# q8888620002/Group-Attribution-for-Diffusion-Models

Measured on AMD Instinct MI355X. Metric: shapley_coalitions_per_hour, higher is better.
Workload: dtype f32; 1 GPU; CIFAR-20 DDPM sFT coalition (BASELINE configs[1]): gd_steps=1000 @B=128 + 10240 samples x 100 DDIM steps @B=32 (32 batches fused/launch), UNet2DModel widths [128, 256, 256, 256] 35.75M params fp32; step = 1/1000 coalition = 1 train step + 1 sampler step @B=1024, enqueued on 3 HIP streams (the train step belongs to a later coalition: independent work); coalitions_in_flight=3

## Files before the change

group-attribution-for-diffusion-models_amd/csrc/gemm_f32.hip:

```cpp
#include "gad_common.h"
#include "gemm_dev.h"

using namespace gadk;

namespace gadk {
void launch_wino4_fused(const DevArgs& w, int bm, hipStream_t st);
}

namespace {

template <int ROWS, int VEC>
struct LoadKCDense : KCSlots<ROWS> {
  using S = KCSlots<ROWS>;
  const float* base;
  long roff[S::NS];
  unsigned rowmask;
  int kend, k;
  bool kok;
  __device__ void init(const float* b, int ld, int row0, int nrows, int kend_) {
    base = b;
    kend = kend_;
    rowmask = 0;
#pragma unroll
    for (int i = 0; i < S::NS; ++i) {
      int r = row0 + S::row(i);
      bool ok = r < nrows;
      roff[i] = ok ? (long)r * ld : 0;
      rowmask |= (unsigned)ok << i;
    }
  }
  __device__ __forceinline__ void prep(int k0, unsigned& mask) {
    k = k0 + S::kq4();
    kok = k < kend;
    mask = rowmask;
// ... 2470 lines not shown
static bool use_wino_wgrad(const gad_gemm_args* a, WinoWgradPlan* wq) {
  const gad_conv_geom& g = a->g;
  if (!(a->flags & GAD_GEMM_WINO_WGRAD) || (a->flags & (GAD_GEMM_NO_WINO | GAD_GEMM_NO_PATCH | GAD_GEMM_INTERNAL_WINO4))) return false;
  if (a->operand_precision != 0 || a->a_mode != GAD_A_MC || a->b_mode != GAD_B_CONV || a->A2 || a->A_k2 || a->batch > 1) return false;
  if (!same_3x3(g) || (g.Ho & 3) || (g.Wo & 3)) return false;
  if (g.C % 4 != 0 || g.ldx % 4 != 0 || a->M % 4 != 0 || a->lda % 4 != 0 || a->N != 9 * g.C || a->ldc % 4 != 0) return false;
  if ((a->tile_hint != 0 && a->tile_hint != HINT_WINO4) || a->splitk_hint > 0 || a->K % (g.Ho * g.Wo) != 0) return false;
  if (a->alpha != 1.f || a->bias || a->rowadd || a->residual) return false;
  if (!(gad_aligned16(a->A) && gad_aligned16(a->B) && gad_aligned16(a->C))) return false;
  wq->T = (long)a->K / 16;
  wq->wy_bytes = (int64_t)36 * wq->T * a->M * 4;
  wq->v_bytes = (int64_t)36 * wq->T * g.C * 4;
  wq->du_bytes = (int64_t)36 * a->M * g.C * 4;
  wq->bytes = wq->wy_bytes + wq->v_bytes + wq->du_bytes;
  if (a->tile_hint == HINT_WINO4) return true;
  const double dy_bytes = 4.0 * a->K * a->M, x_bytes = 4.0 * (double)(a->K / (g.Ho * g.Wo)) * g.H * g.W * g.C;
  const double t_w = (dy_bytes + x_bytes + (double)wq->wy_bytes + (double)wq->v_bytes) / 4.9e12 + 36.0 * wq->T * a->M * (double)g.C * 2.0 / 100e12 +
                     3.0 * (double)wq->du_bytes / 3.0e12 + 30e-6;
  const double t_direct = 2.0 * a->K * (double)a->M * a->N / 115e12;
  return t_w < 0.9 * t_direct;
}


static gad_gemm_args products36(const gad_gemm_args* a, const float* A, const float* B, float* C, int am, int bm, int M, int N, int K) {
  gad_gemm_args sub = *a;
  sub.A = A; sub.B = B; sub.C = C;
  sub.a_mode = am; sub.b_mode = bm;
  sub.M = M; sub.N = N; sub.K = K;
  sub.lda = am == GAD_A_MC ? M : K; sub.ldb = bm == GAD_B_MC ? N : K; sub.ldc = N;
  sub.batch = 36; sub.batch_inner = 1;
  sub.strideA0 = (int64_t)M * K; sub.strideB0 = (int64_t)N * K; sub.strideC0 = (int64_t)M * N;
  sub.strideA1 = sub.strideB1 = sub.strideC1 = 0;
  sub.tile_hint = 0; sub.splitk_hint = 0;
  sub.flags = GAD_GEMM_INTERNAL_WINO4;
  sub.B_wino = nullptr; sub.B_wino4 = nullptr; sub.wino_ws = nullptr; sub.wino_ws_bytes = 0;
  sub.A2 = nullptr;
  return sub;
}
static gad_gemm_args wino_wgrad_products_args(const gad_gemm_args* a, const WinoWgradPlan& wq, float* Wy, float* V, float* dU) {
  return products36(a, Wy, V, dU, GAD_A_MC, GAD_B_MC, a->M, a->g.C, (int)wq.T);
}
static gad_gemm_args wino4_products_args(const gad_gemm_args* a, const WinoPlan& wp, float* V, float* Mb) {
  gad_gemm_args sub = products36(a, V, a->B_wino4, Mb, GAD_A_KC, GAD_B_KC, (int)wp.T, a->N, a->g.C);
  sub.alpha = 1.f; sub.bias = nullptr; sub.rowadd = nullptr; sub.residual = nullptr;
  return sub;
}

enum class RouteKind { ENGINE, PATCH_F32, PATCH_BF16, FEWOUT, WGRAD_PATCH, WINO, WINO_WGRAD, SPLIT_N, SPLIT_M };
struct Route {
  RouteKind kind;
  gad_gemm_args a;
  int vec;
  bool bf16;
  Plan plan;
  PatchPlan pp;
  WinoPlan wp;
  WinoWgradPlan wq;
  int wbm, wsplits;
  int split;
};

static Route route_of(const gad_gemm_args* args) {
  Route r{};
  r.a = canonical(args);
  const gad_gemm_args* a = &r.a;
  r.vec = pick_vec(a);
  r.bf16 = use_bf16(a);
  if (use_wino_wgrad(a, &r.wq)) r.kind = RouteKind::WINO_WGRAD;
  else if (use_wino(a, &r.wp)) r.kind = RouteKind::WINO;
  else if (patch_split_n(a, &r.split)) {
    r.kind = RouteKind::SPLIT_N;
    use_patch_conv_f32(a, &r.pp);
  } else if (wgrad_split_m(a, &r.split)) {
    r.kind = RouteKind::SPLIT_M;
    r.wsplits = wgrad_patch_splits(a, &r.wbm);
  } else if (use_fewout_conv(a)) r.kind = RouteKind::FEWOUT;
  else if ((r.wsplits = wgrad_patch_splits(a, &r.wbm))) r.kind = RouteKind::WGRAD_PATCH;
  else if (use_patch_conv(a)) r.kind = RouteKind::PATCH_BF16;
  else if (use_patch_conv_f32(a, &r.pp)) r.kind = RouteKind::PATCH_F32;
  else {
    r.kind = RouteKind::ENGINE;
    r.plan = make_plan(a);
  }
  return r;
}

struct Report { int kid, tile, splitk; };
static Report report(const Route& r) {
  switch (r.kind) {
    case RouteKind::ENGINE: return {r.bf16 ? 1 : 0, r.plan.bm, r.plan.splitk};
    case RouteKind::PATCH_F32: return {2, r.pp.bn, r.pp.splitk};
    case RouteKind::SPLIT_N: return {2, 224, r.pp.splitk};
    case RouteKind::SPLIT_M: return {2, 224, r.wsplits};
    case RouteKind::WGRAD_PATCH: return {2, r.wbm, r.wsplits};
    case RouteKind::PATCH_BF16: return {3, 128, 1};
    case RouteKind::FEWOUT: return {4, 256, 1};
    case RouteKind::WINO: return {r.wp.f == 2 ? 5 : 6, r.wp.f == 2 ? r.wp.bn : (r.wp.fused4 == 2 ? r.wp.bm : 128), 1};
    case RouteKind::WINO_WGRAD: return {7, 128, 1};
  }
  return {-1, 0, 0};
}

static void split_halves(const Route& r, gad_gemm_args* lo, gad_gemm_args* hi) {
  const gad_gemm_args* a = &r.a;
  const int s = r.split;
  *lo = *a;
  *hi = *a;
  if (r.kind == RouteKind::SPLIT_M) {
    if (a->tile_hint >= HINT_SPLIT_M) lo->tile_hint = hi->tile_hint = 0;
    lo->M = s;
    hi->M = a->M - s;
    hi->A = a->A + s;
    hi->C = a->C + (long)s * a->ldc;
    return;
  }
  lo->B_wino = lo->B_wino4 = hi->B_wino = hi->B_wino4 = nullptr;
  lo->wino_ws = hi->wino_ws = nullptr;
  lo->wino_ws_bytes = hi->wino_ws_bytes = 0;
  lo->N = s;
  hi->N = a->N - s;
  hi->B = a->B + (long)s * a->ldb;
  hi->C = a->C + s;
  if (a->bias) hi->bias = a->bias + s;
  if (a->rowadd) hi->rowadd = a->rowadd + s;
  if (a->residual) hi->residual = a->residual + s;
}

static int64_t workspace_bytes(const Route& r) {
  const gad_gemm_args* a = &r.a;
  switch (r.kind) {
    case RouteKind::ENGINE: case RouteKind::PATCH_F32: case RouteKind::WGRAD_PATCH: case RouteKind::PATCH_BF16: case RouteKind::FEWOUT: {
      const int splitk = report(r).splitk;
      return splitk > 1 ? (int64_t)(a->batch > 0 ? a->batch : 1) * splitk * a->M * a->N * (int64_t)sizeof(float) : 0;
    }
    case RouteKind::WINO: {
      if (r.wp.f == 2 || r.wp.fused4) return 0;
      const gad_gemm_args sub = wino4_products_args(a, r.wp, nullptr, nullptr);
      return gad_gemm_workspace_bytes(&sub);
    }
    case RouteKind::WINO_WGRAD: {
      const gad_gemm_args sub = wino_wgrad_products_args(a, r.wq, nullptr, nullptr, nullptr);
      return gad_gemm_workspace_bytes(&sub);
    }
    case RouteKind::SPLIT_N: case RouteKind::SPLIT_M: {
      gad_gemm_args lo, hi;
      split_halves(r, &lo, &hi);
      const int64_t wl = gad_gemm_workspace_bytes(&lo), wh = gad_gemm_workspace_bytes(&hi);
      return wl > wh ? wl : wh;
    }
  }
  return 0;
}

extern "C" int gad_gemm_uses_bf16(const gad_gemm_args* a) { return a && route_of(a).bf16 ? 1 : 0; }

extern "C" int gad_gemm_kernel_id(const gad_gemm_args* a) { return a ? report(route_of(a)).kid : -1; }

extern "C" int gad_gemm_plan(const gad_gemm_args* a, int32_t* tile, int32_t* splitk, int32_t* vec) {
  GAD_CHECK(a && tile && splitk && vec, "gad_gemm_plan: null pointer");
  const Route r = route_of(a);
  const Report rep = report(r);
  *tile = rep.tile;
  *splitk = rep.splitk;
  *vec = r.vec;
  return 0;
}

extern "C" int64_t gad_gemm_wino_bytes(const gad_gemm_args* a) {
  if (!a) return 0;
  const Route r = route_of(a);
  return r.kind == RouteKind::WINO ? r.wp.bytes : r.kind == RouteKind::WINO_WGRAD ? r.wq.bytes : 0;
}

extern "C" int64_t gad_gemm_workspace_bytes(const gad_gemm_args* a) { return a ? workspace_bytes(route_of(a)) : 0; }

extern "C" int gad_wino_weights(const float* src, float* dst, const int64_t* table, int64_t n_tiles, void* stream) {
// ... 384 lines not shown
  GAD_CASE(GAD_A_MC, GAD_B_MC)
  GAD_CASE(GAD_A_CONV, GAD_B_KC)
  GAD_CASE(GAD_A_CONVT, GAD_B_WDGRAD)
  GAD_CASE(GAD_A_MC, GAD_B_CONV)
  {
    gad_set_error("gad_gemm: unsupported mode pair a_mode=%d b_mode=%d", am, bmode);
    return 1;
  }
#undef GAD_CASE
  GAD_LAUNCH_CHECK("gad_gemm");
  if (pl.splitk > 1) {
    launch_splitk_reduce(d, (int)batch, st);
    GAD_LAUNCH_CHECK("gad_gemm(splitk reduce)");
  }
  return 0;
}

extern "C" int gad_gemm(const gad_gemm_args* args, void* stream) {
  GAD_CHECK(args && args->A && args->B && args->C, "gad_gemm: null pointer");
  const gad_gemm_args canon = canonical(args);
  if (const int rc = check_args(&canon)) return rc;
  const Route r = route_of(&canon);
  if (const int rc = check_stage_flags(r)) return rc;
  hipStream_t st = (hipStream_t)stream;
  DevArgs d = dev_args(&r.a);
  switch (r.kind) {
    case RouteKind::SPLIT_N: case RouteKind::SPLIT_M: {
      gad_gemm_args lo, hi;
      split_halves(r, &lo, &hi);
      const int rc = gad_gemm(&lo, stream);
      return rc ? rc : gad_gemm(&hi, stream);
    }
    case RouteKind::WINO_WGRAD: return launch_wino_wgrad(r, stream);
    case RouteKind::WINO: return launch_wino(r, d, stream);
    case RouteKind::FEWOUT: return launch_fewout(r, d, st);
    case RouteKind::WGRAD_PATCH: return launch_wgrad_patch(r, d, st);
    case RouteKind::PATCH_BF16: return launch_patch_bf16(r, d, st);
    case RouteKind::PATCH_F32: return launch_patch_f32(r, d, st);
    case RouteKind::ENGINE: return launch_engine(r, d, st);
  }
  return 1;
}
```

group-attribution-for-diffusion-models_amd/gad/_capi.py:

```python
import ctypes as C
import os

_HERE = os.path.dirname(os.path.abspath(__file__))
LIB_PATH = os.path.join(_HERE, "libgad_hip.so")


class GadError(RuntimeError):
    pass


class ConvGeom(C.Structure):
    _fields_ = [("H", C.c_int32), ("W", C.c_int32), ("C", C.c_int32), ("ldx", C.c_int32),
                ("Ho", C.c_int32), ("Wo", C.c_int32), ("KH", C.c_int32), ("KW", C.c_int32),
                ("stride", C.c_int32), ("pad_t", C.c_int32), ("pad_l", C.c_int32), ("upsample", C.c_int32)]


class GemmArgs(C.Structure):
    _fields_ = [("A", C.c_void_p), ("B", C.c_void_p), ("C", C.c_void_p),
                ("a_mode", C.c_int32), ("b_mode", C.c_int32),
                ("M", C.c_int32), ("N", C.c_int32), ("K", C.c_int32),
                ("lda", C.c_int32), ("ldb", C.c_int32), ("ldc", C.c_int32),
                ("batch", C.c_int32), ("batch_inner", C.c_int32),
                ("strideA0", C.c_int64), ("strideA1", C.c_int64), ("strideB0", C.c_int64),
                ("strideB1", C.c_int64), ("strideC0", C.c_int64), ("strideC1", C.c_int64),
# ... 48 lines not shown
                ("ws", C.c_void_p), ("ws_bytes", C.c_int64),
                ("tile_hint", C.c_int32), ("splitk_hint", C.c_int32)]


class AdamArgs(C.Structure):
    _fields_ = [("p", C.c_void_p), ("g", C.c_void_p), ("m", C.c_void_p), ("v", C.c_void_p), ("ema", C.c_void_p),
                ("n", C.c_int64), ("sumsq", C.c_void_p), ("max_norm", C.c_float),
                ("lr", C.c_float), ("beta1", C.c_float), ("beta2", C.c_float), ("eps", C.c_float),
                ("weight_decay", C.c_float), ("adamw", C.c_int32), ("step", C.c_int32), ("ema_decay", C.c_float)]


class JLArgs(C.Structure):
    _fields_ = [("A", C.c_void_p), ("lda", C.c_int64), ("G", C.c_int32), ("P", C.c_int64), ("p0", C.c_int64),
                ("d", C.c_int32), ("seed", C.c_uint32), ("model_id", C.c_uint32), ("type", C.c_int32),
                ("accumulate", C.c_int32), ("out", C.c_void_p), ("workspace", C.c_void_p), ("workspace_bytes", C.c_int64)]


class HGemmSegArgs(C.Structure):
    _fields_ = [("A", C.c_void_p), ("B", C.c_void_p), ("C", C.c_void_p), ("ws", C.c_void_p), ("ws_bytes", C.c_int64),
                ("c_seg_stride", C.c_int64), ("M", C.c_int32), ("N", C.c_int32), ("L", C.c_int32), ("S", C.c_int32),
                ("lda", C.c_int32), ("ldb", C.c_int32), ("ldc", C.c_int32), ("alpha", C.c_float), ("accumulate", C.c_int32),
                ("splitk_hint", C.c_int32)]


JL_NORMAL, JL_RADEMACHER = 0, 1
POOL_MAX, POOL_AVG, POOL_AVG_VALID = 0, 1, 2
GELU_ERF, GELU_QUICK = 0, 1
SIM_X_F32, SIM_X_U8 = 0, 1

GEMM_NO_PATCH, GEMM_TAP_MAJOR_K, GEMM_SCALAR_EPILOGUE, GEMM_GENERAL_LOADERS, GN_TWO_PASS = 1, 2, 4, 8, 1
GEMM_NO_WINO = 16
GEMM_WINO_WGRAD = 32
GEMM_WINO_ONLY_INPUT, GEMM_WINO_SKIP_INPUT = 64, 128
A_KC, A_MC, A_CONV, A_CONVT = 0, 1, 2, 3
B_KC, B_MC, B_WDGRAD, B_CONV = 0, 1, 2, 3

_vp, _i32, _i64, _f32, _f64 = C.c_void_p, C.c_int32, C.c_int64, C.c_float, C.c_double

SIGNATURES = {
    "gad_version": (C.c_int, []),
    "gad_last_error": (C.c_char_p, []),
    "gad_gemm_workspace_bytes": (_i64, [C.POINTER(GemmArgs)]),
    "gad_gemm": (C.c_int, [C.POINTER(GemmArgs), _vp]),
    "gad_gemm_uses_bf16": (C.c_int, [C.POINTER(GemmArgs)]),
    "gad_gemm_kernel_id": (C.c_int, [C.POINTER(GemmArgs)]),
    "gad_gemm_wino_bytes": (_i64, [C.POINTER(GemmArgs)]),
    "gad_wino_weights": (C.c_int, [_vp, _vp, _vp, _i64, _vp]),
    "gad_wino4_weights": (C.c_int, [_vp, _vp, _vp, _i64, _vp]),
    "gad_groupnorm_one_pass": (C.c_int, [C.POINTER(GroupNormArgs)]),
    "gad_gemm_plan": (C.c_int, [C.POINTER(GemmArgs), C.POINTER(_i32), C.POINTER(_i32), C.POINTER(_i32)]),
    "gad_groupnorm_workspace_bytes": (_i64, [C.POINTER(GroupNormArgs)]),
    "gad_groupnorm_silu_fwd": (C.c_int, [C.POINTER(GroupNormArgs), _vp]),
    "gad_groupnorm_silu_bwd": (C.c_int, [C.POINTER(GroupNormArgs), _vp]),
    "gad_groupnorm_wino4_ok": (C.c_int, [C.POINTER(GroupNormArgs), C.c_int32]),
    "gad_groupnorm_silu_wino4": (C.c_int, [C.POINTER(GroupNormArgs), _vp, C.c_int32, _vp]),
    "gad_attention_supported": (C.c_int, [_i32]),
    "gad_attention_uses_bf16": (C.c_int, [C.POINTER(AttentionArgs), _i32]),
    "gad_attention_bwd_workspace_bytes": (_i64, [C.POINTER(AttentionArgs)]),
    "gad_attention_fwd": (C.c_int, [C.POINTER(AttentionArgs), _vp]),
    "gad_attention_bwd": (C.c_int, [C.POINTER(AttentionArgs), _vp]),
    "gad_attention_d512_supported": (C.c_int, [_i32]),
    "gad_attention_fwd_d512": (C.c_int, [C.POINTER(AttentionArgs), _vp]),
    "gad_attention_causal_supported": (C.c_int, [_i32, _i32]),
    "gad_attention_causal_fwd": (C.c_int, [C.POINTER(AttentionArgs), _vp]),
    "gad_softmax_fwd": (C.c_int, [_vp, _vp, _i64, _i32, _f32, _vp]),
    "gad_softmax_bwd": (C.c_int, [_vp, _vp, _vp, _i64, _i32, _f32, _vp]),
# ... 96 lines not shown
```

group-attribution-for-diffusion-models_amd/gad/ops.py:

```python
from __future__ import annotations

import ctypes as C
import math
from typing import Optional

import torch

from . import _capi
from ._capi import (A_CONV, A_CONVT, A_KC, A_MC, B_CONV, B_KC, B_MC, B_WDGRAD, AdamArgs, ConvGeom, GemmArgs,
                    GroupNormArgs, check)
from .shadows import (WEIGHT_EPOCH, Shadow, cached, in_flat_buffer as _in_flat_buffer, weight_key, written,
                      written_everywhere)

_WS = {}
WS_BYTES = 1 << 30


def _stream():
    return C.c_void_p(torch.cuda.current_stream().cuda_stream)


_raw_stream = getattr(torch._C, "_cuda_getCurrentRawStream", None)


# ... 121 lines not shown
        KERNEL_FLAGS["no_wino4"] = self.no_wino4
        KERNEL_FLAGS["no_gn_wino"] = self.no_gn_wino
        return self

    def __exit__(self, *exc):
        KERNEL_FLAGS.update(self.prev)
        return False


SCRATCH_ALLOC = None
OUT_ALLOC = None
OUT_ALLOC_DT = None


ROUTE_STATS = None


def _scratch(kind, nbytes, device):
    if SCRATCH_ALLOC is not None:
        return SCRATCH_ALLOC(kind, nbytes, device)
    return torch.empty(nbytes, dtype=torch.uint8, device=device)


def _out(shape, device):
    if OUT_ALLOC is not None:
        return OUT_ALLOC(tuple(shape), device)
    return torch.empty(tuple(shape), device=device, dtype=torch.float32)


def gemm_raw(A, B, Cout, a_mode, b_mode, M, N, K, lda, ldb, ldc, *, geom: Optional[ConvGeom] = None, alpha=1.0,
             bias=None, rowadd=None, rows_per_group=1, residual=None, ldr=0, batch=1, batch_inner=1,
             sA=(0, 0), sB=(0, 0), sC=(0, 0), tile_hint=0, splitk_hint=0, A2=None, a_split=0, B_bf16=None,
             A_k2=None, B_k2=None, k_split=0, B_wino=None, B_wino4=None, wino_wgrad=False, wino_input=None, force_f32=False,
             keep_v=None, wino_v=None):
    lib = _capi.load()
    ws = workspace(A.device)
    a = GemmArgs()
    a.A, a.B, a.C = A.data_ptr(), B.data_ptr(), Cout.data_ptr()
    a.a_mode, a.b_mode = a_mode, b_mode
    a.M, a.N, a.K = M, N, K
    a.lda, a.ldb, a.ldc = lda, ldb, ldc
    a.batch, a.batch_inner = batch, batch_inner
    a.strideA0, a.strideA1 = sA
    a.strideB0, a.strideB1 = sB
    a.strideC0, a.strideC1 = sC
    if geom is not None:
        a.g = geom
    a.alpha = alpha
    a.bias, a.rowadd, a.residual = _ptr(bias), _ptr(rowadd), _ptr(residual)
    a.rows_per_group = rows_per_group
    a.ld_rowadd = (rowadd.stride(0) if rowadd.ndim == 2 else rowadd.shape[-1]) if rowadd is not None else 0
    a.ldr = ldr
    a.ws, a.ws_bytes = ws.data_ptr(), ws.numel()
    a.tile_hint, a.splitk_hint = tile_hint, splitk_hint
    a.operand_precision = 1 if (OPERAND_PRECISION[0] and not force_f32) else 0
    a.flags = KERNEL_FLAGS["gemm"]
    if A2 is not None:
        a.A2, a.a_split, a.ldx2 = A2.data_ptr(), a_split, A2.shape[-1]
    if B_bf16 is not None:
        a.B_bf16 = B_bf16.data_ptr()
    if A_k2 is not None:
        a.A_k2, a.B_k2, a.k_split = A_k2.data_ptr(), B_k2.data_ptr(), k_split
        a.lda_k2, a.ldb_k2 = A_k2.shape[-1], B_k2.shape[-1]
    if B_wino is not None or B_wino4 is not None:
        a.B_wino, a.B_wino4 = _ptr(B_wino), _ptr(B_wino4)
        need = lib.gad_gemm_wino_bytes(C.byref(a))
        if need:
            V = _scratch("wino", need, A.device)
            a.wino_ws, a.wino_ws_bytes = V.data_ptr(), need
            if keep_v is not None and a.B_wino4 and lib.gad_gemm_kernel_id(C.byref(a)) == 6:
                keep_v.append(V)
        else:
            a.B_wino = a.B_wino4 = None
    if wino_wgrad:
        a.flags |= _capi.GEMM_WINO_WGRAD
        need = lib.gad_gemm_wino_bytes(C.byref(a))
        if need:
            V = _scratch("wino", need, A.device)
            a.wino_ws, a.wino_ws_bytes = V.data_ptr(), need
            if wino_v is not None and wino_v.numel() >= 36 * (K // 16) * geom.C * 4:
                a.B_wino4 = wino_v.data_ptr()
                a.flags |= _capi.GEMM_WINO_SKIP_INPUT
        else:
            a.flags &= ~_capi.GEMM_WINO_WGRAD
    if wino_input is not None:
        if lib.gad_gemm_kernel_id(C.byref(a)) != 6 or not a.wino_ws:
            return False
        wino_input(V)
        a.flags |= _capi.GEMM_WINO_SKIP_INPUT
# ... 6 lines not shown
        a.ws, a.ws_bytes = (ws.data_ptr() if need else None), need
    if PROFILER is not None:
        PROFILER.gemm(lib, a, batch)
        return True
    check(lib.gad_gemm(C.byref(a), _stream()), "gad_gemm")
    return True


class GemmProfiler:
    NAMES = {(A_CONV, B_KC): "conv_fwd", (A_CONVT, B_WDGRAD): "conv_dgrad", (A_MC, B_CONV): "conv_wgrad",
             (A_KC, B_KC): "gemm_nt", (A_KC, B_MC): "gemm_nn", (A_MC, B_MC): "gemm_tn"}

    def __init__(self):
        self.records = []

    def gemm(self, lib, a, batch):
        tile, sk, vec = C.c_int32(), C.c_int32(), C.c_int32()
        check(lib.gad_gemm_plan(C.byref(a), C.byref(tile), C.byref(sk), C.byref(vec)), "gad_gemm_plan")
        kid = lib.gad_gemm_kernel_id(C.byref(a))
        s, e, mid = torch.cuda.Event(enable_timing=True), torch.cuda.Event(enable_timing=True), None
        s.record()
        if kid in (5, 6) and not (a.flags & _capi.GEMM_WINO_SKIP_INPUT):
            flags = a.flags
            mid = torch.cuda.Event(enable_timing=True)
            a.flags = flags | _capi.GEMM_WINO_ONLY_INPUT
            check(lib.gad_gemm(C.byref(a), _stream()), "gad_gemm")
            mid.record()
            a.flags = flags | _capi.GEMM_WINO_SKIP_INPUT
            check(lib.gad_gemm(C.byref(a), _stream()), "gad_gemm")
            a.flags = flags
        else:
            check(lib.gad_gemm(C.byref(a), _stream()), "gad_gemm")
        e.record()
        name = self.NAMES.get((a.a_mode, a.b_mode), "gemm") + ("", "_bf16", f"_patch_w{a.g.Wo}", f"_patch_bf16_w{a.g.Wo}", f"_fewout_valu_w{a.g.Wo}", "_wino", "_wino4", "_wino4")[kid]
        key = (name, tile.value, sk.value, vec.value)
        g = a.g
        if a.a_mode in (A_CONV, A_CONVT):
            a_elems = (a.M // max(1, g.Ho * g.Wo)) * g.H * g.W * g.C
        else:
            a_elems = a.M * a.K
        b_elems = (a.K // max(1, g.Ho * g.Wo)) * g.H * g.W * g.C if a.b_mode == B_CONV else a.N * a.K
        extra = a.M * a.N if a.residual else 0
        nbytes = 4.0 * max(1, batch) * (a_elems + b_elems + a.M * a.N + extra)
        flops = 2.0 * a.M * a.N * a.K * max(1, batch)
        executed = flops * ({5: 16.0 / 36.0, 6: 0.25, 7: 0.25}.get(kid, 1.0))
        stage = None
        if kid in (5, 6):
            npos, tpx = (16, 4) if kid == 5 else (36, 16)
            v_bytes = 4.0 * npos * (a.M // tpx) * g.C
            stage = (mid, 4.0 * a_elems + v_bytes if mid is not None else 0.0, v_bytes + 4.0 * (b_elems * npos / 9.0 + a.M * a.N + extra))
        self.records.append((key, flops, nbytes, s, e, executed, stage))

    def hgemm(self, lib, a, tn=False):
        s, e = torch.cuda.Event(enable_timing=True), torch.cuda.Event(enable_timing=True)
        if tn:
            s.record()
            check(lib.gad_hgemm_tn(C.byref(a), _stream()), "gad_hgemm_tn")
            e.record()
            nbytes = 2.0 * a.K * (a.M + a.N) + 4.0 * a.M * a.N
            flops = 2.0 * a.M * a.N * a.K
            self.records.append((("hgemm_tn_wgrad", 128, 0, 8), flops, nbytes, s, e, flops, None))
            return
        tile, sk = C.c_int32(), C.c_int32()
        check(lib.gad_hgemm_plan(C.byref(a), C.byref(tile), C.byref(sk)), "gad_hgemm_plan")
        s.record()
        check(lib.gad_hgemm(C.byref(a), _stream()), "gad_hgemm")
        e.record()
# ... 236 lines not shown
    _req(dy, "conv dy")
    Bn, H, W, Cin = x_shape
    wk = weight_krsc(w)
    Cout, KH, KW, _ = wk.shape
    _, Ho, Wo, _ = dy.shape
    He, We = (2 * H, 2 * W) if upsample else (H, W)
    dxe = _out((Bn, He, We, Cin), dy.device)
    if (KH == 1 and KW == 1 and stride == 1 and tuple(pad) == (0, 0, 0, 0) and not upsample and Cin % 4 == 0 and Cout % 4 == 0
            and not KERNEL_FLAGS["gemm"] & _capi.GEMM_GENERAL_LOADERS):
        gemm_raw(dy, wk, dxe, A_KC, B_MC, Bn * H * W, Cin, Cout, Cout, Cin, Cin, tile_hint=tile_hint, splitk_hint=splitk_hint)
        return dxe
    g = ConvGeom(Ho, Wo, Cout, Cout, He, We, KH, KW, stride, pad[0], pad[2], 0)
    gemm_raw(dy, wk, dxe, A_CONVT, B_WDGRAD, Bn * He * We, Cin, KH * KW * Cout, 0, 0, Cin, geom=g,
             tile_hint=tile_hint, splitk_hint=splitk_hint)
    return _upsample2x_bwd(dxe, x_shape) if upsample else dxe


def _upsample2x_bwd(dxe, x_shape):
    Bn, H, W, Cin = x_shape
    dx = torch.empty((Bn, H, W, Cin), device=dxe.device, dtype=torch.float32)
    check(_capi.load().gad_upsample2x_bwd(dxe.data_ptr(), dx.data_ptr(), Bn, H, W, Cin, _stream()), "gad_upsample2x_bwd")
    return dx


def conv2d_wgrad_raw(dy, x, w_like, stride=1, pad=(1, 1, 1, 1), upsample=False, tile_hint=0, splitk_hint=0, out=None, wino_v=None):
    _req(dy, "conv dy")
    _req(x, "conv x")
    Bn, H, W, Cin = x.shape
    Cout, _, KH, KW = w_like.shape
    _, Ho, Wo, _ = dy.shape
    dwk = _out((Cout, KH, KW, Cin), dy.device) if out is None else weight_krsc(out)
    if (KH == 1 and KW == 1 and stride == 1 and tuple(pad) == (0, 0, 0, 0) and not upsample and Cin % 4 == 0 and Cout % 4 == 0
            and not KERNEL_FLAGS["gemm"] & _capi.GEMM_GENERAL_LOADERS):
        gemm_raw(dy, x, dwk, A_MC, B_MC, Cout, Cin, Bn * H * W, Cout, Cin, Cin, tile_hint=tile_hint, splitk_hint=splitk_hint)
        return dwk.permute(0, 3, 1, 2)
    g = ConvGeom(H, W, Cin, Cin, Ho, Wo, KH, KW, stride, pad[0], pad[2], int(upsample))
    wino = (KH == 3 and KW == 3 and stride == 1 and tuple(pad) == (1, 1, 1, 1) and tile_hint in (0, 8) and splitk_hint == 0
            and Ho % 4 == 0 and Wo % 4 == 0 and OPERAND_PRECISION[0] == 0 and not KERNEL_FLAGS.get("no_wino4")
            and not KERNEL_FLAGS["gemm"] & (_capi.GEMM_NO_WINO | _capi.GEMM_NO_PATCH | _capi.GEMM_SCALAR_EPILOGUE | _capi.GEMM_TAP_MAJOR_K
                                            | _capi.GEMM_GENERAL_LOADERS))
    gemm_raw(dy, x, dwk, A_MC, B_CONV, Cout, KH * KW * Cin, Bn * Ho * Wo, Cout, 0, KH * KW * Cin, geom=g,
             tile_hint=tile_hint, splitk_hint=splitk_hint, wino_wgrad=wino, wino_v=wino_v)
    return dwk.permute(0, 3, 1, 2)


def colsum_raw(dy2d: torch.Tensor, segments=1, out=None):
    lib = _capi.load()
    ws = workspace(dy2d.device)
    rows, N = dy2d.shape
    if out is None:
        out = torch.empty((segments, N), device=dy2d.device, dtype=torch.float32)
    check(lib.gad_colsum(dy2d.data_ptr(), out.data_ptr(), segments, rows // segments, N, ws.data_ptr(), ws.numel(),
                         _stream()), "gad_colsum")
    return out


def linear_fwd_raw(x2d, w, bias=None, residual=None, alpha=1.0, force_f32=False):
    M, K = x2d.shape
    N = w.shape[0]
    y = _out((M, N), x2d.device)
    gemm_raw(x2d, w, y, A_KC, B_KC, M, N, K, K, K, N, bias=bias, residual=residual, ldr=N, alpha=alpha, force_f32=force_f32)
    return y


def conv_krsc_raw(x, w_krsc, bias, kh, kw, stride, pad_h, pad_w, out=None, c0=0):
    Bn, H, W, ci = x.shape
    co = w_krsc.shape[0]
# ... 129 lines not shown
    if z2d.dtype != torch.float32 or codebook.dtype != torch.float32 or not codebook.is_contiguous() or (D > 1 and z2d.stride(1) != 1):
        raise _capi.GadError("vq_lookup: fp32 rows with unit column stride and a contiguous fp32 codebook are required")
    if codebook.ndim != 2 or codebook.shape[1] != D:
        raise _capi.GadError(f"vq_lookup: codebook {tuple(codebook.shape)} does not hold codes of {D}")
    idx = torch.empty((n,), device=z2d.device, dtype=torch.int32)
    zq = torch.empty((n, D), device=z2d.device, dtype=torch.float32)
    check(_capi.load().gad_vq_lookup(z2d.data_ptr(), z2d.stride(0) if n > 1 else D, codebook.data_ptr(), n, codebook.shape[0], D,
                                     idx.data_ptr(), zq.data_ptr(), D, _stream()), "gad_vq_lookup")
    return idx, zq


def layernorm_fwd_raw(x, gamma, beta, eps):
    C_ = x.shape[-1]
    rows = x.numel() // C_
    y = torch.empty_like(x)
    stats = torch.empty((2, rows), device=x.device, dtype=torch.float32)
    check(_capi.load().gad_layernorm_fwd(x.data_ptr(), y.data_ptr(), gamma.data_ptr(), beta.data_ptr(), stats[0].data_ptr(),
                                         stats[1].data_ptr(), rows, C_, eps, _stream()), "gad_layernorm_fwd")
    return y, stats[0], stats[1]


def linear_dgrad_raw(dy2d, w):
    M, N = dy2d.shape
    K = w.shape[1]
    dx = _out((M, K), dy2d.device)
    gemm_raw(dy2d, w, dx, A_KC, B_MC, M, K, N, N, K, K)
    return dx


def linear_wgrad_raw(dy2d, x2d, out=None):
    M, N = dy2d.shape
    K = x2d.shape[1]
    dw = _out((N, K), dy2d.device) if out is None else out
    gemm_raw(dy2d, x2d, dw, A_MC, B_MC, N, K, M, N, K, K)
    return dw


def _param_grad(param, compute):
    v, first = _sink(param)
    if v is None:
        return compute(None)
    if first:
        compute(v)
    else:
        v.add_(compute(None))
    return None


def _conv_backward(ctx, dy, x, x_shape, w, stride, pad, upsample, has, need):
    dy = dy.contiguous()
    dx = None
    if need[0]:
        if dgrad_as_forward(w, stride, pad):
            dx = conv2d_fwd_raw(dy, rotated_weight(w), None)
            if upsample:
                dx = _upsample2x_bwd(dx, x_shape)
        else:
            dx = conv2d_dgrad_raw(dy, w, x_shape, stride, pad, upsample)
    V, ctx.wino_v = ctx.wino_v, None
    dw = _param_grad(w, lambda o: conv2d_wgrad_raw(dy, x, w, stride, pad, upsample, out=o, wino_v=V)) if need[1] else None
    db, dr = _conv_epilogue_grads(dy, ctx.bias_ref, has[0] and need[2], has[1] and need[3])
    dres = dy if (has[2] and need[4]) else None
    return dx, dw, db, dr, dres


class Conv2dFn(torch.autograd.Function):

# ... 819 lines not shown
```

include/gad.h:

```cpp
#ifndef GAD_H
#define GAD_H
#include <stdint.h>
#ifdef __cplusplus
extern "C" {
#endif

int gad_version(void);
const char* gad_last_error(void);

enum gad_a_mode {
  GAD_A_KC = 0,
  GAD_A_MC = 1,
  GAD_A_CONV = 2,
  GAD_A_CONVT = 3
};
enum gad_b_mode {
  GAD_B_KC = 0,
  GAD_B_MC = 1,
  GAD_B_WDGRAD = 2,
  GAD_B_CONV = 3
};

typedef struct gad_conv_geom {
  int32_t H, W, C;
// ... 16 lines not shown
  int64_t strideA0, strideA1, strideB0, strideB1, strideC0, strideC1;
  gad_conv_geom g;
  float alpha;
  const float* bias;
  const float* rowadd;
  int32_t rows_per_group, ld_rowadd;
  const float* residual;
  int32_t ldr;
  void* ws;
  int64_t ws_bytes;
  int32_t tile_hint;
  int32_t splitk_hint;
  int32_t operand_precision;
  const float* A2;
  int32_t a_split, ldx2;
  const void* B_bf16;
  const float* A_k2;
  const float* B_k2;
  int32_t lda_k2, ldb_k2, k_split;
  int32_t flags;
  const float* B_wino;
  void* wino_ws;
  int64_t wino_ws_bytes;
  const float* B_wino4;
} gad_gemm_args;
enum gad_gemm_flags {
  GAD_GEMM_NO_WINO = 16,
  GAD_GEMM_WINO_WGRAD = 32,
  GAD_GEMM_NO_PATCH = 1,
  GAD_GEMM_TAP_MAJOR_K = 2,
  GAD_GEMM_SCALAR_EPILOGUE = 4,
  GAD_GEMM_GENERAL_LOADERS = 8,
  GAD_GEMM_WINO_ONLY_INPUT = 64,
  GAD_GEMM_WINO_SKIP_INPUT = 128
};

int64_t gad_gemm_workspace_bytes(const gad_gemm_args* a);
int gad_gemm_plan(const gad_gemm_args* a, int32_t* tile, int32_t* splitk, int32_t* vec);
int gad_gemm(const gad_gemm_args* a, void* stream);
int gad_gemm_uses_bf16(const gad_gemm_args* a);
int gad_gemm_kernel_id(const gad_gemm_args* a);
int64_t gad_gemm_wino_bytes(const gad_gemm_args* a);
int gad_wino_weights(const float* src, float* dst, const int64_t* table, int64_t n_tiles, void* stream);
int gad_wino4_weights(const float* src, float* dst, const int64_t* table, int64_t n_tiles, void* stream);

typedef struct gad_groupnorm_args {
  const float* x;
  float* y;
  const float* gamma;
  const float* beta;
  float* mean;
  float* rstd;
  const float* dy;
  float* dgamma;
  float* dbeta;
  int32_t B, HW, C, G;
  float eps;
  int32_t silu;
  void* ws;
  int64_t ws_bytes;
  const float* x2;
  int32_t C1;
  int32_t flags;
  const float* dx_add;
} gad_groupnorm_args;
enum gad_groupnorm_flags { GAD_GN_TWO_PASS = 1 };

// ... 225 lines not shown
```

Baseline: 46.09 coalitions/hour.

## Add split-K slab MFMA kernel for long-K TN weight-gradient GEMMs

Adds a new TN GEMM route for weight-gradient GEMMs (both operands M/N-contiguous along a very long K reduction). It uses 128x128 tiles with f32 MFMA and double-buffered LDS, splits K into slabs written to workspace, then sums them in a separate reduce kernel. The route is opted into by 1x1 conv wgrad, linear wgrad and the Winograd wgrad products, and is gated by a size heuristic. The aim is more parallelism and better tensor-core use on skinny-output, long-K GEMMs. The cost is an extra workspace pass and reduce launch.

```diff
diff --git a/group-attribution-for-diffusion-models_amd/csrc/gemm_f32.hip b/group-attribution-for-diffusion-models_amd/csrc/gemm_f32.hip
--- a/group-attribution-for-diffusion-models_amd/csrc/gemm_f32.hip
+++ b/group-attribution-for-diffusion-models_amd/csrc/gemm_f32.hip
@@ -1,5 +1,6 @@
 #include "gad_common.h"
 #include "gemm_dev.h"
+#include "wgrad_tn.h"
 
 using namespace gadk;
 
@@ -2536,7 +2537,7 @@
   sub.strideA0 = (int64_t)M * K; sub.strideB0 = (int64_t)N * K; sub.strideC0 = (int64_t)M * N;
   sub.strideA1 = sub.strideB1 = sub.strideC1 = 0;
   sub.tile_hint = 0; sub.splitk_hint = 0;
-  sub.flags = GAD_GEMM_INTERNAL_WINO4;
+  sub.flags = GAD_GEMM_INTERNAL_WINO4 | (a->flags & GAD_GEMM_TN_SLAB);
   sub.B_wino = nullptr; sub.B_wino4 = nullptr; sub.wino_ws = nullptr; sub.wino_ws_bytes = 0;
   sub.A2 = nullptr;
   return sub;
@@ -2550,7 +2551,21 @@
   return sub;
 }
 
-enum class RouteKind { ENGINE, PATCH_F32, PATCH_BF16, FEWOUT, WGRAD_PATCH, WINO, WINO_WGRAD, SPLIT_N, SPLIT_M };
+static bool use_tn_slab(const gad_gemm_args* a, TnSlabPlan* tp) {
+  if (!(a->flags & GAD_GEMM_TN_SLAB) || (a->flags & ~(GAD_GEMM_TN_SLAB | GAD_GEMM_INTERNAL_WINO4))) return false;
+  if (a->a_mode != GAD_A_MC || a->b_mode != GAD_B_MC || a->operand_precision != 0 || a->tile_hint != 0) return false;
+  if (a->bias || a->rowadd || a->residual || a->A2 || a->A_k2 || a->B_k2) return false;
+  if (a->M <= 0 || a->N <= 0 || a->K <= 0 || a->M % 4 != 0 || a->N % 4 != 0 || a->lda % 4 != 0 || a->ldb % 4 != 0 || a->ldc % 4 != 0) return false;
+  if (a->lda < a->M || a->ldb < a->N || a->ldc < a->N) return false;
+  if (!(gad_aligned16(a->A) && gad_aligned16(a->B) && gad_aligned16(a->C))) return false;
+  if (a->batch > 1 && (a->strideA0 % 4 != 0 || a->strideA1 % 4 != 0 || a->strideB0 % 4 != 0 || a->strideB1 % 4 != 0 ||
+                       a->strideC0 % 4 != 0 || a->strideC1 % 4 != 0)) return false;
+  if (a->splitk_hint <= 0 && !tn_slab_gate(a->M, a->N, a->K, a->batch)) return false;
+  *tp = tn_slab_plan(a->M, a->N, a->K, a->batch, a->splitk_hint);
+  return true;
+}
+
+enum class RouteKind { ENGINE, PATCH_F32, PATCH_BF16, FEWOUT, WGRAD_PATCH, WINO, WINO_WGRAD, SPLIT_N, SPLIT_M, TN_SLAB };
 struct Route {
   RouteKind kind;
   gad_gemm_args a;
@@ -2562,6 +2577,7 @@
   WinoWgradPlan wq;
   int wbm, wsplits;
   int split;
+  TnSlabPlan tn;
 };
 
 static Route route_of(const gad_gemm_args* args) {
@@ -2570,7 +2586,8 @@
   const gad_gemm_args* a = &r.a;
   r.vec = pick_vec(a);
   r.bf16 = use_bf16(a);
-  if (use_wino_wgrad(a, &r.wq)) r.kind = RouteKind::WINO_WGRAD;
+  if (use_tn_slab(a, &r.tn)) r.kind = RouteKind::TN_SLAB;
+  else if (use_wino_wgrad(a, &r.wq)) r.kind = RouteKind::WINO_WGRAD;
   else if (use_wino(a, &r.wp)) r.kind = RouteKind::WINO;
   else if (patch_split_n(a, &r.split)) {
     r.kind = RouteKind::SPLIT_N;
@@ -2601,6 +2618,7 @@
     case RouteKind::FEWOUT: return {4, 256, 1};
     case RouteKind::WINO: return {r.wp.f == 2 ? 5 : 6, r.wp.f == 2 ? r.wp.bn : (r.wp.fused4 == 2 ? r.wp.bm : 128), 1};
     case RouteKind::WINO_WGRAD: return {7, 128, 1};
+    case RouteKind::TN_SLAB: return {8, TN_TILE, r.tn.slabs};
   }
   return {-1, 0, 0};
 }
@@ -2646,6 +2664,8 @@
       const gad_gemm_args sub = wino_wgrad_products_args(a, r.wq, nullptr, nullptr, nullptr);
       return gad_gemm_workspace_bytes(&sub);
     }
+    case RouteKind::TN_SLAB:
+      return r.tn.slabs > 1 ? (int64_t)r.tn.slabs * (a->batch > 0 ? a->batch : 1) * a->M * a->N * (int64_t)sizeof(float) : 0;
     case RouteKind::SPLIT_N: case RouteKind::SPLIT_M: {
       gad_gemm_args lo, hi;
       split_halves(r, &lo, &hi);
@@ -3096,6 +3116,7 @@
       return rc ? rc : gad_gemm(&hi, stream);
     }
     case RouteKind::WINO_WGRAD: return launch_wino_wgrad(r, stream);
+    case RouteKind::TN_SLAB: return tn_slab_launch(&r.a, r.tn, st);
     case RouteKind::WINO: return launch_wino(r, d, stream);
     case RouteKind::FEWOUT: return launch_fewout(r, d, st);
     case RouteKind::WGRAD_PATCH: return launch_wgrad_patch(r, d, st);
diff --git a/group-attribution-for-diffusion-models_amd/csrc/wgrad_tn.h b/group-attribution-for-diffusion-models_amd/csrc/wgrad_tn.h
--- /dev/null
+++ b/group-attribution-for-diffusion-models_amd/csrc/wgrad_tn.h
@@ -0,0 +1,19 @@
+#pragma once
+#include "gad_common.h"
+
+namespace gadk {
+
+constexpr int TN_TILE = 128;
+constexpr int TN_KS = 16;
+
+struct TnSlabPlan {
+  int tiles_m, tiles_n;
+  int slabs;
+  int steps_per_slab;
+};
+
+TnSlabPlan tn_slab_plan(int M, int N, int K, int batch, int splitk_hint);
+bool tn_slab_gate(int M, int N, int K, int batch);
+int tn_slab_launch(const gad_gemm_args* a, const TnSlabPlan& pl, hipStream_t st);
+
+}
diff --git a/group-attribution-for-diffusion-models_amd/csrc/wgrad_tn.hip b/group-attribution-for-diffusion-models_amd/csrc/wgrad_tn.hip
--- /dev/null
+++ b/group-attribution-for-diffusion-models_amd/csrc/wgrad_tn.hip
@@ -0,0 +1,242 @@
+#include "wgrad_tn.h"
+
+#include <type_traits>
+
+namespace gadk {
+
+struct TnArgs {
+  const float* A;
+  const float* B;
+  float* C;
+  float* ws;
+  int M, N, K;
+  int lda, ldb, ldc;
+  int batch, batch_inner;
+  long sA0, sA1, sB0, sB1, sC0, sC1;
+  int tiles_m, tiles_n, slabs, steps_per_slab;
+  float alpha;
+  int groups;
+};
+
+static __device__ __forceinline__ f32x4 tn_ldg4(const float* p) { return *reinterpret_cast<const f32x4*>(p); }
+
+__global__ __launch_bounds__(256, 2) void tn_slab_kernel(const TnArgs p) {
+  __shared__ __attribute__((aligned(16))) float As[2][TN_KS][TN_TILE];
+  __shared__ __attribute__((aligned(16))) float Bs[2][TN_KS][TN_TILE];
+  const int tid = threadIdx.x, lane = tid & 63, wave = tid >> 6;
+  const int wm = wave >> 1, wn = wave & 1;
+  const int tiles = p.tiles_m * p.tiles_n;
+  int bid = blockIdx.x;
+  const int tile = bid % tiles;
+  bid /= tiles;
+  const int slab = bid % p.slabs, z = bid / p.slabs;
+  const int m0 = (tile % p.tiles_m) * TN_TILE, n0 = (tile / p.tiles_m) * TN_TILE;
+  const int z0 = z / p.batch_inner, z1 = z - z0 * p.batch_inner;
+  const float* Ab = p.A + z0 * p.sA0 + z1 * p.sA1;
+  const float* Bb = p.B + z0 * p.sB0 + z1 * p.sB1;
+
+  const long k0 = (long)slab * p.steps_per_slab * TN_KS;
+  long kend = k0 + (long)p.steps_per_slab * TN_KS;
+  if (kend > p.K) kend = p.K;
+  const int nsteps = (int)((kend - k0 + TN_KS - 1) / TN_KS);
+
+  const int r0 = tid >> 5, c = (tid & 31) * 4;
+  const bool a_ok = m0 + c < p.M, b_ok = n0 + c < p.N;
+  const float* pa[2] = {Ab + (k0 + r0) * p.lda + m0 + c, Ab + (k0 + r0 + 8) * p.lda + m0 + c};
+  const float* pb[2] = {Bb + (k0 + r0) * p.ldb + n0 + c, Bb + (k0 + r0 + 8) * p.ldb + n0 + c};
+  const long step_a = (long)TN_KS * p.lda, step_b = (long)TN_KS * p.ldb;
+  long tok = k0 + r0;
+
+  f32x4 va[2][2], vb[2][2];
+  int mask[2];
+  auto load = [&](auto set) {
+    constexpr int S = decltype(set)::value;
+    mask[S] = 0;
+#pragma unroll
+    for (int i = 0; i < 2; ++i) {
+      const bool in = tok + 8 * i < kend;
+      const bool ia = in && a_ok, ib = in && b_ok;
+      va[S][i] = tn_ldg4(ia ? pa[i] : Ab);
+      vb[S][i] = tn_ldg4(ib ? pb[i] : Bb);
+      mask[S] |= (ia ? 1 : 0) << (2 * i) | (ib ? 2 : 0) << (2 * i);
+      pa[i] += step_a;
+      pb[i] += step_b;
+    }
+    tok += TN_KS;
+  };
+  auto stage = [&](int buf, auto set) {
+    constexpr int S = decltype(set)::value;
+#pragma unroll
+    for (int i = 0; i < 2; ++i) {
+      *reinterpret_cast<f32x4*>(&As[buf][r0 + 8 * i][c]) = (mask[S] >> (2 * i) & 1) ? va[S][i] : f32x4{0.f, 0.f, 0.f, 0.f};
+      *reinterpret_cast<f32x4*>(&Bs[buf][r0 + 8 * i][c]) = (mask[S] >> (2 * i) & 2) ? vb[S][i] : f32x4{0.f, 0.f, 0.f, 0.f};
+    }
+  };
+
+  f32x16 acc[2][2];
+#pragma unroll
+  for (int i = 0; i < 2; ++i)
+#pragma unroll
+    for (int j = 0; j < 2; ++j)
+#pragma unroll
+      for (int r = 0; r < 16; ++r) acc[i][j][r] = 0.f;
+
+  const int fr = lane & 31, fk = lane >> 5;
+  auto step = [&](auto set) {
+    constexpr int S = decltype(set)::value;
+    load(set);
+    const float* ar = &As[S][fk][wm * 64 + fr];
+    const float* br = &Bs[S][fk][wn * 64 + fr];
+    float a0 = ar[0], a1 = ar[32], b0 = br[0], b1 = br[32];
+#pragma unroll
+    for (int kk = 0; kk < TN_KS / 2; ++kk) {
+      float na0 = 0.f, na1 = 0.f, nb0 = 0.f, nb1 = 0.f;
+      if (kk + 1 < TN_KS / 2) {
+        na0 = ar[(2 * kk + 2) * TN_TILE]; na1 = ar[(2 * kk + 2) * TN_TILE + 32];
+        nb0 = br[(2 * kk + 2) * TN_TILE]; nb1 = br[(2 * kk + 2) * TN_TILE + 32];
+      }
+      __builtin_amdgcn_sched_barrier(0);
+      acc[0][0] = __builtin_amdgcn_mfma_f32_32x32x2f32(a0, b0, acc[0][0], 0, 0, 0);
+      acc[0][1] = __builtin_amdgcn_mfma_f32_32x32x2f32(a0, b1, acc[0][1], 0, 0, 0);
+      acc[1][0] = __builtin_amdgcn_mfma_f32_32x32x2f32(a1, b0, acc[1][0], 0, 0, 0);
+      acc[1][1] = __builtin_amdgcn_mfma_f32_32x32x2f32(a1, b1, acc[1][1], 0, 0, 0);
+      a0 = na0; a1 = na1; b0 = nb0; b1 = nb1;
+    }
+    if constexpr (S == 0) stage(1, std::integral_constant<int, 1>{});
+    else stage(0, std::integral_constant<int, 0>{});
+    __syncthreads();
+  };
+  load(std::integral_constant<int, 0>{});
+  load(std::integral_constant<int, 1>{});
+  stage(0, std::integral_constant<int, 0>{});
+  __syncthreads();
+  for (int s = 0; s < nsteps; s += 2) {
+    step(std::integral_constant<int, 0>{});
+    step(std::integral_constant<int, 1>{});
+  }
+
+  const bool direct = p.slabs == 1;
+  float* out;
+  long ld;
+  if (direct) {
+    out = p.C + z0 * p.sC0 + z1 * p.sC1;
+    ld = p.ldc;
+  } else {
+    out = p.ws + ((long)slab * p.batch + z) * ((long)p.M * p.N);
+    ld = p.N;
+  }
+#pragma unroll
+  for (int i = 0; i < 2; ++i)
+#pragma unroll
+    for (int j = 0; j < 2; ++j) {
+      const int n = n0 + wn * 64 + j * 32 + fr;
+#pragma unroll
+      for (int r = 0; r < 16; ++r) {
+        const int m = m0 + wm * 64 + i * 32 + (r & 3) + 8 * (r >> 2) + 4 * fk;
+        if (m < p.M && n < p.N) out[(long)m * ld + n] = direct ? p.alpha * acc[i][j][r] : acc[i][j][r];
+      }
+    }
+}
+
+template <int W>
+__global__ __launch_bounds__(256) void tn_slab_reduce_kernel(const TnArgs p) {
+  typedef float vec_t __attribute__((ext_vector_type(W)));
+  __shared__ __attribute__((aligned(16))) float part[256 * W];
+  const long mn = (long)p.M * p.N, total = (long)p.batch * mn;
+  const int per_block = 256 / p.groups;
+  const int o = threadIdx.x % per_block, g = threadIdx.x / per_block;
+  const long idx = ((long)blockIdx.x * per_block + o) * W;
+  const bool live = idx < total;
+  const int chunk = (p.slabs + p.groups - 1) / p.groups;
+  const int s0 = g * chunk, s1 = s0 + chunk < p.slabs ? s0 + chunk : p.slabs;
+  vec_t v = 0.f;
+  if (live && s0 < s1) {
+    const float* src = p.ws + idx;
+    v = *reinterpret_cast<const vec_t*>(src + (long)s0 * total);
+    int s = s0 + 1;
+    for (; s + 4 <= s1; s += 4) {
+      const vec_t t0 = *reinterpret_cast<const vec_t*>(src + (long)s * total), t1 = *reinterpret_cast<const vec_t*>(src + (long)(s + 1) * total);
+      const vec_t t2 = *reinterpret_cast<const vec_t*>(src + (long)(s + 2) * total), t3 = *reinterpret_cast<const vec_t*>(src + (long)(s + 3) * total);
+      v += t0; v += t1; v += t2; v += t3;
+    }
+    for (; s < s1; ++s) v += *reinterpret_cast<const vec_t*>(src + (long)s * total);
+  }
+  if (p.groups > 1) {
+    *reinterpret_cast<vec_t*>(&part[threadIdx.x * W]) = v;
+    __syncthreads();
+    if (g == 0)
+      for (int h = 1; h < p.groups; ++h)
+        if (h * chunk < p.slabs) v += *reinterpret_cast<const vec_t*>(&part[(h * per_block + o) * W]);
+  }
+  if (live && g == 0) {
+    const int z = (int)(idx / mn);
+    const long r = idx - (long)z * mn;
+    const int m = (int)(r / p.N), n = (int)(r - (long)m * p.N);
+    const int z0 = z / p.batch_inner, z1 = z - z0 * p.batch_inner;
+    *reinterpret_cast<vec_t*>(p.C + z0 * p.sC0 + z1 * p.sC1 + (long)m * p.ldc + n) = v * p.alpha;
+  }
+}
+
+TnSlabPlan tn_slab_plan(int M, int N, int K, int batch, int splitk_hint) {
+  TnSlabPlan pl;
+  pl.tiles_m = (int)gad_ceil_div(M, TN_TILE);
+  pl.tiles_n = (int)gad_ceil_div(N, TN_TILE);
+  const long tiles = (long)pl.tiles_m * pl.tiles_n * (batch > 0 ? batch : 1);
+  const long ksteps = gad_ceil_div(K, TN_KS) > 0 ? gad_ceil_div(K, TN_KS) : 1;
+  long want;
+  if (splitk_hint > 0) want = splitk_hint;
+  else {
+    want = 512 / tiles;
+    if (want > ksteps / 8) want = ksteps / 8;
+  }
+  if (want > ksteps) want = ksteps;
+  if (want < 1) want = 1;
+  pl.steps_per_slab = (int)gad_ceil_div(ksteps, want);
+  if (pl.steps_per_slab > 1) pl.steps_per_slab += pl.steps_per_slab & 1;
+  pl.slabs = (int)gad_ceil_div(ksteps, pl.steps_per_slab);
+  return pl;
+}
+
+bool tn_slab_gate(int M, int N, int K, int batch) {
+  const TnSlabPlan pl = tn_slab_plan(M, N, K, batch, 0);
+  const long tiles = (long)pl.tiles_m * pl.tiles_n;
+  if (batch > 1) return K >= 8192 * tiles;
+  const long area = tiles * TN_TILE * TN_TILE;
+  return tiles * pl.slabs >= 480 && ((K >= 4096 * tiles && 4L * M * N >= 3 * area) || (K >= 32768 * tiles && 2L * M * N >= area));
+}
+
+int tn_slab_launch(const gad_gemm_args* a, const TnSlabPlan& pl, hipStream_t st) {
+  const int batch = a->batch > 0 ? a->batch : 1;
+  const long blocks = (long)pl.tiles_m * pl.tiles_n * pl.slabs * batch;
+  GAD_CHECK(blocks > 0 && blocks < (1L << 31), "gad_gemm(tn slab): grid too large");
+  GAD_CHECK(a->lda >= a->M && a->ldb >= a->N && a->ldc >= a->N, "gad_gemm(tn slab): leading dimension below the row length");
+  TnArgs p;
+  p.A = a->A; p.B = a->B; p.C = a->C; p.ws = (float*)a->ws;
+  p.M = a->M; p.N = a->N; p.K = a->K;
+  p.lda = a->lda; p.ldb = a->ldb; p.ldc = a->ldc;
+  p.batch = batch; p.batch_inner = a->batch_inner > 0 ? a->batch_inner : 1;
+  p.sA0 = a->strideA0; p.sA1 = a->strideA1; p.sB0 = a->strideB0; p.sB1 = a->strideB1; p.sC0 = a->strideC0; p.sC1 = a->strideC1;
+  if (batch == 1) p.sA0 = p.sA1 = p.sB0 = p.sB1 = p.sC0 = p.sC1 = 0;
+  p.tiles_m = pl.tiles_m; p.tiles_n = pl.tiles_n; p.slabs = pl.slabs; p.steps_per_slab = pl.steps_per_slab;
+  p.alpha = a->alpha;
+  const bool vec = gad_aligned16(a->ws);
+  const long outputs = (long)batch * a->M * a->N / (vec ? 4 : 1);
+  p.groups = 1;
+  while (p.groups < 16 && p.groups * 2 <= pl.slabs && outputs * p.groups < 65536) p.groups *= 2;
+  if (pl.slabs > 1) {
+    const int64_t need = (int64_t)pl.slabs * batch * a->M * a->N * (int64_t)sizeof(float);
+    GAD_CHECK(a->ws && a->ws_bytes >= need, "gad_gemm(tn slab): workspace too small (%lld < %lld)", (long long)a->ws_bytes, (long long)need);
+  }
+  hipLaunchKernelGGL(tn_slab_kernel, dim3((unsigned)blocks), dim3(256), 0, st, p);
+  GAD_LAUNCH_CHECK("gad_gemm(tn slab)");
+  if (pl.slabs > 1) {
+    const long rb = gad_ceil_div(outputs, 256 / p.groups);
+    GAD_CHECK(rb < (1L << 31), "gad_gemm(tn slab reduce): grid too large");
+    if (vec) hipLaunchKernelGGL(tn_slab_reduce_kernel<4>, dim3((unsigned)rb), dim3(256), 0, st, p);
+    else hipLaunchKernelGGL(tn_slab_reduce_kernel<1>, dim3((unsigned)rb), dim3(256), 0, st, p);
+    GAD_LAUNCH_CHECK("gad_gemm(tn slab reduce)");
+  }
+  return 0;
+}
+
+}
diff --git a/group-attribution-for-diffusion-models_amd/gad/_capi.py b/group-attribution-for-diffusion-models_amd/gad/_capi.py
--- a/group-attribution-for-diffusion-models_amd/gad/_capi.py
+++ b/group-attribution-for-diffusion-models_amd/gad/_capi.py
@@ -104,6 +104,7 @@
 GEMM_NO_WINO = 16
 GEMM_WINO_WGRAD = 32
 GEMM_WINO_ONLY_INPUT, GEMM_WINO_SKIP_INPUT = 64, 128
+GEMM_TN_SLAB = 256
 A_KC, A_MC, A_CONV, A_CONVT = 0, 1, 2, 3
 B_KC, B_MC, B_WDGRAD, B_CONV = 0, 1, 2, 3
 
diff --git a/group-attribution-for-diffusion-models_amd/gad/ops.py b/group-attribution-for-diffusion-models_amd/gad/ops.py
--- a/group-attribution-for-diffusion-models_amd/gad/ops.py
+++ b/group-attribution-for-diffusion-models_amd/gad/ops.py
@@ -177,7 +177,7 @@
              bias=None, rowadd=None, rows_per_group=1, residual=None, ldr=0, batch=1, batch_inner=1,
              sA=(0, 0), sB=(0, 0), sC=(0, 0), tile_hint=0, splitk_hint=0, A2=None, a_split=0, B_bf16=None,
              A_k2=None, B_k2=None, k_split=0, B_wino=None, B_wino4=None, wino_wgrad=False, wino_input=None, force_f32=False,
-             keep_v=None, wino_v=None):
+             keep_v=None, wino_v=None, tn_slab=False):
     lib = _capi.load()
     ws = workspace(A.device)
     a = GemmArgs()
@@ -200,6 +200,8 @@
     a.tile_hint, a.splitk_hint = tile_hint, splitk_hint
     a.operand_precision = 1 if (OPERAND_PRECISION[0] and not force_f32) else 0
     a.flags = KERNEL_FLAGS["gemm"]
+    if (tn_slab or wino_wgrad) and a.operand_precision == 0:
+        a.flags |= _capi.GEMM_TN_SLAB
     if A2 is not None:
         a.A2, a.a_split, a.ldx2 = A2.data_ptr(), a_split, A2.shape[-1]
     if B_bf16 is not None:
@@ -272,7 +274,7 @@
         else:
             check(lib.gad_gemm(C.byref(a), _stream()), "gad_gemm")
         e.record()
-        name = self.NAMES.get((a.a_mode, a.b_mode), "gemm") + ("", "_bf16", f"_patch_w{a.g.Wo}", f"_patch_bf16_w{a.g.Wo}", f"_fewout_valu_w{a.g.Wo}", "_wino", "_wino4", "_wino4")[kid]
+        name = self.NAMES.get((a.a_mode, a.b_mode), "gemm") + ("", "_bf16", f"_patch_w{a.g.Wo}", f"_patch_bf16_w{a.g.Wo}", f"_fewout_valu_w{a.g.Wo}", "_wino", "_wino4", "_wino4", "_slab")[kid]
         key = (name, tile.value, sk.value, vec.value)
         g = a.g
         if a.a_mode in (A_CONV, A_CONVT):
@@ -575,7 +577,8 @@
     dwk = _out((Cout, KH, KW, Cin), dy.device) if out is None else weight_krsc(out)
     if (KH == 1 and KW == 1 and stride == 1 and tuple(pad) == (0, 0, 0, 0) and not upsample and Cin % 4 == 0 and Cout % 4 == 0
             and not KERNEL_FLAGS["gemm"] & _capi.GEMM_GENERAL_LOADERS):
-        gemm_raw(dy, x, dwk, A_MC, B_MC, Cout, Cin, Bn * H * W, Cout, Cin, Cin, tile_hint=tile_hint, splitk_hint=splitk_hint)
+        gemm_raw(dy, x, dwk, A_MC, B_MC, Cout, Cin, Bn * H * W, Cout, Cin, Cin, tile_hint=tile_hint, splitk_hint=splitk_hint,
+                 tn_slab=tile_hint == 0 and splitk_hint == 0)
         return dwk.permute(0, 3, 1, 2)
     g = ConvGeom(H, W, Cin, Cin, Ho, Wo, KH, KW, stride, pad[0], pad[2], int(upsample))
     wino = (KH == 3 and KW == 3 and stride == 1 and tuple(pad) == (1, 1, 1, 1) and tile_hint in (0, 8) and splitk_hint == 0
@@ -771,7 +774,7 @@
     M, N = dy2d.shape
     K = x2d.shape[1]
     dw = _out((N, K), dy2d.device) if out is None else out
-    gemm_raw(dy2d, x2d, dw, A_MC, B_MC, N, K, M, N, K, K)
+    gemm_raw(dy2d, x2d, dw, A_MC, B_MC, N, K, M, N, K, K, tn_slab=True)
     return dw
 
 
diff --git a/include/gad.h b/include/gad.h
--- a/include/gad.h
+++ b/include/gad.h
@@ -72,7 +72,8 @@
   GAD_GEMM_SCALAR_EPILOGUE = 4,
   GAD_GEMM_GENERAL_LOADERS = 8,
   GAD_GEMM_WINO_ONLY_INPUT = 64,
-  GAD_GEMM_WINO_SKIP_INPUT = 128
+  GAD_GEMM_WINO_SKIP_INPUT = 128,
+  GAD_GEMM_TN_SLAB = 256
 };
 
 int64_t gad_gemm_workspace_bytes(const gad_gemm_args* a);
```

Result: no change. 45.69 coalitions/hour (-0.9%).
